# srtweezer/RobustGRAPE

Measured on AMD Instinct MI355X. Metric: GRAPE gradient-evals/sec (fidelity+∇), Rydberg CZ d=9 N_t=512, 1→8 GPU, higher is better.
Workload: dtype f64

## Files before the change

### robustgrape_amd/csrc/grape_call.hip

```cpp
#include <hip/hip_runtime.h>

#include <algorithm>
#include <cstring>
#include <string>
#include <vector>

#include "grape_plan.hpp"

using namespace grape_eng;

namespace grape_eng {

static grape_dense::DenseBatch dense_batch(grape_plan *p, int nb, const double *d_x, double *d_F, double *d_Fdx,
                                           double *d_Fd2, double *d_Fd2dx) {
    grape_dense::DenseBatch DB{};
    DB.nb = nb;
    DB.x = d_x;
    DB.E = p->dn_E;
    DB.Q = p->dn_Q;
    DB.Carry = p->dn_Carry;
    DB.M = p->dn_M;
    DB.Mc = p->dn_Mc;
    DB.Z = p->dn_Z;
    DB.Ub = p->dn_Ub;
// ... 69 lines not shown
        FA.Fd2dx = P.ne ? d_Fd2dx + (size_t)b * P.ne * nx : nullptr;
        HIPCHECK(grape_unitary::launch_fidelity(FA, st));
        mk(GRAPE_KERNEL_GRAD, 1);
    }
    return GRAPE_OK;
}

static KMark profiling_mark(grape_plan *p) {
    KMark mk;
    if (p->profiling) {
        mk.ctx = p;
        mk.fn = [](void *ctx, int k, int phase) {
            grape_plan *pl = static_cast<grape_plan *>(ctx);
            hipEvent_t e = pl->get_event();
            if (!e) return;
            (void)hipEventRecord(e, pl->cur_stream);
            if (phase == 0) {
                pl->pending.push_back({k, e, nullptr});
            } else {
                pl->pending.back().b = e;
            }
        };
    }
    return mk;
}

static int enqueue_wide(grape_plan *p, int nb, const double *d_x, double *d_F, double *d_Fdx) {
    hipStream_t st = p->stream;
    p->cur_stream = st;
    const KMark mk = profiling_mark(p);
    const int ma = p->merge_pa, mb = 1 - ma;
    DevProblem Pw[2] = {p->Ps[ma], p->Ps[mb]};
    DevBatch Bw[2]{};
    grape_proj::SectorHead H = p->SH;
    for (int i = 0; i < 2; ++i) {
        const int cl = i == 0 ? ma : mb;
        const grape_plan::SecBuf &sb = p->sb[cl];
        Pw[i].nchunks = 1;
        Pw[i].L = Pw[i].Nt;
        Bw[i].nb = nb * Pw[i].nsec;
        Bw[i].x = d_x;
        Bw[i].F = d_F;
        Bw[i].Fdx = d_Fdx;
        Bw[i].Ub = sb.Tc;
        Bw[i].Msec = sb.Carry;
        Bw[i].status = p->d_ctrl + 2;
        Bw[i].sink = p->d_sink;
        H.Ub[cl] = sb.Tc;
        H.Msec[cl] = sb.Carry;
    }
    H.alpha = 1;
    H.x = d_x;
    H.F = d_F;
    H.Fdx = d_Fdx;
    H.tgt_part = p->d_tgt_part;
    mk(GRAPE_KERNEL_WALK_FWD, 0);
    HIPCHECK(grape_walk::launch_merged_wide(0, Pw[0], Bw[0], Pw[1], Bw[1], st));
    mk(GRAPE_KERNEL_WALK_FWD, 1);
    mk(GRAPE_KERNEL_SCAN, 0);
    HIPCHECK(grape_proj::launch_sector_head(H, nb, st));
    mk(GRAPE_KERNEL_SCAN, 1);
    mk(GRAPE_KERNEL_WALK_GRAD, 0);
    HIPCHECK(grape_walk::launch_merged_wide(1, Pw[0], Bw[0], Pw[1], Bw[1], st));
    mk(GRAPE_KERNEL_WALK_GRAD, 1);
    return GRAPE_OK;
}

static int enqueue(grape_plan *p, int nb, const double *d_x, double *d_F, double *d_Fdx, double *d_Fd2,
                   double *d_Fd2dx) {
    hipStream_t st = p->stream;
    p->cur_stream = st;
    const KMark mk = profiling_mark(p);
    if (p->tiled) {
        grape_tiled::TiledBatch TB = p->TB;
        TB.nb = nb;
        TB.x = d_x;
        TB.F = d_F;
        TB.Fdx = d_Fdx;
        HIPCHECK(grape_tiled::launch_pipeline(p->TP, TB, st, mk));
        return GRAPE_OK;
    }
    if (p->general_h0) return enqueue_general(p, nb, d_x, d_F, d_Fdx, d_Fd2, d_Fd2dx, mk);
    if (p->dense) {
        const grape_dense::DenseBatch DB = dense_batch(p, nb, d_x, d_F, d_Fdx, d_Fd2, d_Fd2dx);
        HIPCHECK(grape_dense::launch_pipeline(p->DP, DB, st, mk));
        return GRAPE_OK;
    }
    if (p->e1) {
        mk(GRAPE_KERNEL_EVAL1, 0);
        HIPCHECK(grape_eval1::launch(eval1_args(p, d_x, d_F, d_Fdx), nb, st));
        mk(GRAPE_KERNEL_EVAL1, 1);
        return GRAPE_OK;
    }
// ... 509 lines not shown
```

### robustgrape_amd/csrc/grape_plan.hpp

```cpp
#pragma once
#include <hip/hip_runtime.h>

#include <string>
#include <vector>

#include "grape.h"
#include "grape_launch_api.hpp"
#include "grape_walk_api.hpp"
#include "grape_projector_api.hpp"
#include "grape_dense_api.hpp"
#include "grape_tiled_api.hpp"
#include "grape_unitary_api.hpp"
#include "grape_eval1_api.hpp"
#include "grape_plan_setup.hpp"
#include "grape_descriptor.hpp"

using grape::DevBatch;
using grape::DevProblem;
using grape::Term;
using grape_host::KMark;

#define HIPCHECK(expr)                                                                  \
    do {                                                                                \
        hipError_t e_ = (expr);                                                         \
// ... 63 lines not shown
    grape::FactorTab FT{};
    Term *d_fac_h0 = nullptr, *d_fac_err = nullptr;
    double *d_W = nullptr;
    cd *d_E = nullptr, *d_Q = nullptr, *d_Mc = nullptr, *d_Carry = nullptr, *d_Ub = nullptr, *d_Me = nullptr;
    grape::VSpec *d_vs = nullptr;
    int *d_ovf2 = nullptr;
    cd *d_ovf2_slots = nullptr;
    double *d_Fd2 = nullptr, *d_Fd2dx = nullptr, *d_part_err = nullptr;
    cd *d_Zl = nullptr;
    double *d_x = nullptr, *d_F = nullptr, *d_Fdx = nullptr, *d_part = nullptr, *d_tgt_part = nullptr;
    int *d_ovf = nullptr, *d_ctrl = nullptr;
    bool tables = false;
    cd *d_Htab = nullptr, *d_U0tab = nullptr;
    cd *d_sink = nullptr;
    cd *d_PA = nullptr, *d_PB = nullptr, *d_P0g = nullptr, *d_gpscr = nullptr;
    struct SecBuf {
        cd *E = nullptr, *Q = nullptr, *Mc = nullptr, *Carry = nullptr, *Ub = nullptr, *slots = nullptr,
           *ops = nullptr, *opsT = nullptr, *Msec = nullptr, *Tc = nullptr, *wscr = nullptr, *Ew = nullptr,
           *gEt = nullptr;
        int *ovf = nullptr, *ovf2 = nullptr, *sidx = nullptr, *gauge_n = nullptr;
        double *part = nullptr;
        cd *Zl = nullptr, *Me = nullptr, *TotS = nullptr, *MsecE = nullptr, *Wc = nullptr;
        double *part_err = nullptr;
    };
    int ncls = 0;
    DevProblem Ps[2]{};
    SecBuf sb[2];
    int *d_fixed = nullptr;
    grape_proj::SectorHead SH{};
    bool e1 = false;
    bool merged = false;
    int merge_pa = 0;
    int wide = 0;
    cd *d_e1_Et = nullptr, *d_e1_scr = nullptr;
    unsigned char *d_e1_tab = nullptr;
    int e1_pa = 0;
    long long *e1_trace = nullptr, *e1_trace_d = nullptr;
    double e1_phase[16] = {0};
    long e1_calls = 0;
    bool symmetry = false;
    cd *d_ops_sym = nullptr, *d_opsT_sym = nullptr, *d_PA_sym = nullptr, *d_PB_sym = nullptr;
    double *d_W_sym = nullptr;
    hipStream_t aux_stream = nullptr;
    hipEvent_t ev_fork = nullptr, ev_join = nullptr;
    bool capturing = false;
    bool dense = false;
    grape_dense::DenseProblem DP{};
    double *dn_opimg = nullptr, *dn_W = nullptr, *dn_E = nullptr, *dn_Q = nullptr, *dn_Carry = nullptr,
           *dn_M = nullptr, *dn_Mc = nullptr, *dn_Z = nullptr, *dn_Ub = nullptr, *dn_Zl = nullptr, *dn_Vc = nullptr,
           *dn_Sx = nullptr, *dn_Tot = nullptr, *dn_Me = nullptr, *dn_Mp = nullptr, *dn_B0 = nullptr,
           *dn_Fadd = nullptr, *dn_Fd2add = nullptr;
    bool tiled = false;
    grape_tiled::TiledProblem TP{};
    grape_tiled::TiledBatch TB{};
    int *tl_h_smax = nullptr;
    grape::VSpec *ud_vs = nullptr;
    cd *ud_E = nullptr, *ud_C = nullptr, *ud_V = nullptr, *ud_S = nullptr, *ud_out = nullptr;
    int *ud_ovf = nullptr;
    cd *ud_gscr = nullptr;
    bool general_h0 = false;
    bool pivot = false;
    cd *ud_Ci = nullptr, *d_G = nullptr;
    cd *d_fscr = nullptr;
    double *ud_Aimg = nullptr;
    std::vector<grape::VSpec> ud_vs_host;
    double *ud_Eimg = nullptr;
// ... 83 lines not shown
```

### robustgrape_amd/csrc/grape_plan_build.hip

```cpp
#include <hip/hip_runtime.h>

#include <algorithm>
#include <climits>
#include <cmath>
#include <cstdlib>
#include <cstring>
#include <string>
#include <vector>

#include "grape_plan.hpp"

namespace grape_eng {

static int merged_chunk_count(long MB, int Nt, int nc, int ncu) {
    if (const char *e = getenv("GRAPE_GAUGE_NCHUNKS")) {
        const int n = atoi(e);
        if (n > 0) return std::min(n, Nt);
    }
    const double simds = 4.0 * ncu;
    double best = 1e300;
    int pick = nc;
    for (int n = std::max(1, nc / 2); n <= std::min(2 * nc, Nt); ++n) {
        const int L = (Nt + n - 1) / n, nch = (Nt + L - 1) / L;
        const double waves = std::ceil((double)MB * nch / 64.0);
// ... 588 lines not shown
    *pb = 1;
    if (p->ncls == 2 && grape_walk::pair_ok(p->Ps[1], p->Ps[0])) std::swap(*pa, *pb);
}

static int setup_merge(PlanBuild &b) {
    grape_plan *p = b.p;
    if (p->ncls != 2) return GRAPE_OK;
    const DevProblem &P = p->P;
    int pa, pb;
    walk_pair_order(p, &pa, &pb);
    DevProblem &A = p->Ps[pa], &Bq = p->Ps[pb];
    if (!(grape_walk::pair_ok(A, Bq) && A.D == 3 && A.gauge && Bq.gauge && A.gauge_a == Bq.gauge_a &&
          A.scan_waves == kScanTiny && Bq.scan_waves == kScanTiny && A.nchunks <= Bq.nchunks && P.np == 1 && P.na <= 1))
        return GRAPE_OK;
    Bq.L = A.L;
    Bq.nchunks = A.nchunks;
    p->merged = !(P.opts & GRAPE_OPT_NO_MERGE) && grape_walk::merged_ok(A, Bq);
    p->merge_pa = pa;
    for (int cl = 0; p->merged && cl < 2; ++cl)
        if (int rc = fill_gauge_table(p, cl, false)) return rc;
    const std::vector<double> &W = b.sps().W;
    bool r1 = p->merged && p->SH.diag && !(P.opts & GRAPE_OPT_NO_RANK1);
    for (int cl = 0; cl < 2; ++cl) {
        const SectorClass &sc = b.ss.cls[cl];
        DevProblem &Pc = p->Ps[cl];
        Pc.rank1 = Pc.rank1_c[0] = Pc.rank1_c[1] = 0;
        r1 = r1 && sc.nsec <= 2;
        for (int w = 0; r1 && w < sc.nsec; ++w) {
            int n = 0;
            for (int r = 0; r < sc.S; ++r) {
                const int g = sc.sidx[(size_t)w * sc.S + r];
                if (g >= 0 && W[g] != 0.0) {
                    Pc.rank1_c[w] = r;
                    ++n;
                }
            }
            r1 = r1 && n == 1;
        }
        if (Pc.twin && grape_walk::merged_twin_sum()) r1 = r1 && Pc.rank1_c[0] == Pc.rank1_c[1];
    }
    A.rank1 = Bq.rank1 = r1 ? 1 : 0;
    const long wide = (long)p->max_batch * A.nchunks;
    if (r1 && !(P.opts & GRAPE_OPT_NO_WIDE) && grape_walk::wide_ok(A, Bq) && wide * 2 <= (long)INT_MAX) p->wide = (int)wide;
    return GRAPE_OK;
}

static int setup_eval1(grape_plan *p) {
    const grape_proj::SectorHead &H = p->SH;
    if (p->ncls != 2 || (long)p->max_batch > kEval1MaxBatch || (p->P.opts & GRAPE_OPT_NO_EVAL1)) return GRAPE_OK;
    int pa, pb;
    walk_pair_order(p, &pa, &pb);
    const DevProblem &A = p->Ps[pa], &Bq = p->Ps[pb];
    if (!grape_walk::pair_ok(A, Bq) || !grape_eval1::eligible(A, Bq, H)) return GRAPE_OK;
    if (p->mem.alloc(&p->d_e1_Et, (size_t)A.D * A.D + 8) != hipSuccess ||
        p->mem.alloc(&p->d_e1_scr, (size_t)2 * 2 * 16) != hipSuccess)
        return fail(GRAPE_ERR_ALLOC, "device allocation failed (eval1)");
    const hipError_t e = grape_eval1::prepare(A, Bq, p->d_e1_Et, p->d_e1_Et + (size_t)A.D * A.D, p->d_e1_scr, p->stream);
    if (e != hipSuccess || hipStreamSynchronize(p->stream) != hipSuccess)
        return fail(GRAPE_ERR_HIP, "eval1 preparation failed");
    p->e1 = true;
    p->e1_pa = pa;
    const size_t tb = grape_eval1::tab_bytes(A, Bq, H);
    if (p->mem.alloc(&p->d_e1_tab, std::max<size_t>(tb, 16)) != hipSuccess)
        return fail(GRAPE_ERR_ALLOC, "device allocation failed (eval1)");
    if (grape_eval1::tab_build(eval1_args(p, nullptr, nullptr, nullptr), p->d_e1_tab, p->stream) != hipSuccess ||
        hipStreamSynchronize(p->stream) != hipSuccess)
        return fail(GRAPE_ERR_HIP, "eval1 table build failed");
    const char *tr = std::getenv("GRAPE_EVAL1_TRACE");
    if (tr && tr[0] == '1' &&
        (hipHostMalloc(reinterpret_cast<void **>(&p->e1_trace), 32 * sizeof(long long), hipHostMallocDefault) != hipSuccess ||
         hipHostGetDevicePointer(reinterpret_cast<void **>(&p->e1_trace_d), p->e1_trace, 0) != hipSuccess))
        return fail(GRAPE_ERR_ALLOC, "eval1 trace buffer");
    return GRAPE_OK;
}

static int setup_sectors(PlanBuild &b) {
// ... 62 lines not shown
```

### robustgrape_amd/csrc/grape_projector.hip

```cpp
#include "grape_kernels.hpp"
#include "grape_projector_api.hpp"

namespace grape_proj {

namespace {

using grape::cd;
using grape::cadd, grape::csub, grape::cscale, grape::cmul, grape::cconj;
constexpr int BLOCK = 256;

template <bool H>
__device__ __forceinline__ cd el(const cd *X, int D, int i, int l) {
    return H ? cconj(X[(size_t)l * D + i]) : X[(size_t)i * D + l];
}

template <bool HA, bool HB>
__device__ void bmm(cd *C, const cd *A, const cd *B, int D) {
    for (int t = threadIdx.x; t < D * D; t += blockDim.x) {
        const int i = t / D, j = t % D;
        cd s{0.0, 0.0};
        for (int l = 0; l < D; ++l) s = cadd(s, cmul(el<HA>(A, D, i, l), el<HB>(B, D, l, j)));
        C[t] = s;
    }
    __syncthreads();
// ... 619 lines not shown
    if (ok && row == 0) H.F[b] = (fsum + tau.re * tau.re + tau.im * tau.im) / P.DD;
    double unused = 0.0;
    cd unused_c{0.0, 0.0};
    if (ok) diag_row_any(H, St, row, el, b, 1, u0, d, tau, unused, unused_c);
    for (int q = 0; q < P.na; ++q) {
        const grape::Pert pq = xadd_pert(P, q);
        __syncthreads();
        if (ok)
            for (int k = row; k < P.n_tgt; k += G) cq[k] = grape::term_coef(St.terms[k], 1, xb, xadd, pq);
        __syncthreads();
        if (ok)
            for (int i = row; i < P.D; i += G) d[i] = cscale(P.inv_eps, csub(target_entry(P, St, cq, i), u0[i]));
        __syncthreads();
        double sa = 0.0;
        cd trd{0.0, 0.0};
        if (ok) diag_row_any(H, St, row, el, b, 2, u0, d, tau, sa, trd);
        sa = group_add(sa, G);
        trd.re = group_add(trd.re, G);
        trd.im = group_add(trd.im, G);
        for (int r = 0; r < H.nfixed; ++r) {
            const int g = St.fixed[r];
            const cd kd = cconj(d[g]), k = cconj(u0[g]);
            sa += St.W[g] * (St.W[g] != 0.0 ? 1.0 : 0.0) * (kd.re * k.re + kd.im * k.im);
            trd = cadd(trd, cscale(St.W[g], kd));
        }
        const double val = (2.0 * sa + 2.0 * (tau.re * trd.re + tau.im * trd.im)) / P.DD;
        if (ok && row == 0) {
            if (P.xadd_dep && H.tgt_part) H.tgt_part[b * P.na + q] = val;
            else H.Fdx[b * P.nx + (size_t)P.np * P.Nt + q] = val;
        }
    }
}

template <int S>
__device__ void err_row(const SectorHead &H, int cl, int w, int r, size_t b, int e, int pass, const cd *u0, const cd *d,
                        cd te, cd *ue, double &t1, double &t2, cd &acc) {
    const grape::DevProblem &P = H.P;
    const int ns = H.nsec[cl], ne = P.ne;
    const double sc = 2.0 / P.DD;
    const size_t bw = b * ns + w;
    const cd *Ub = H.Ub[cl] + bw * S * S;
    int g[S];
#pragma unroll
    for (int k = 0; k < S; ++k) g[k] = H.sidx[cl][w * S + k];
    const int gr = g[r];
    auto cu0 = [&](int k) { return cconj(u0[g[k] >= 0 ? g[k] : 0]); };
    if (pass == 0) {
        const cd *Tb = H.TotS[cl] + (bw * ne + e) * S * S;
        cd Ur[S];
#pragma unroll
        for (int c = 0; c < S; ++c) {
            cd v{0.0, 0.0};
#pragma unroll
            for (int m = 0; m < S; ++m) v = cadd(v, cmul(Ub[r * S + m], Tb[m * S + c]));
            Ur[c] = (gr >= 0 && g[c] >= 0) ? v : cd{0.0, 0.0};
            ue[r * S + c] = Ur[c];
        }
        if (gr < 0) return;
        const double wr = P.W[gr];
#pragma unroll
        for (int c = 0; c < S; ++c) {
            if (g[c] < 0) continue;
            const cd ke = cmul(cu0(r), Ur[c]);
            t1 += wr * pdiag(P, g[c]) * (ke.re * ke.re + ke.im * ke.im);
            t2 += P.W[g[c]] * (Ur[c].re * Ur[c].re + Ur[c].im * Ur[c].im);
        }
// ... 94 lines not shown
        sa = group_add(sa, G);
        trd.re = group_add(trd.re, G);
        trd.im = group_add(trd.im, G);
        if (ok && row == 0)
            H.Fd2dx[(size_t)be * P.nx + (size_t)P.np * P.Nt + q] = 2.0 * (2.0 * sa + 2.0 * (te.re * trd.re + te.im * trd.im)) / P.DD;
    }
}

hipError_t launch_sector_err_head(const SectorHead &H, int nb, hipStream_t st) {
    if (H.P.ne == 0) return hipSuccess;
    if (H.diag) {
        const int G = diag_group(H), EB = kDiagBlock / G, n = nb * H.P.ne;
        const size_t lds = (size_t)EB * err_rows_group_cd(H) * sizeof(cd);
        hipLaunchKernelGGL(k_sec_err_head_rows, dim3((unsigned)((n + EB - 1) / EB)), dim3(kDiagBlock), lds, st, H, nb);
        return hipGetLastError();
    }
    const size_t lds = (size_t)kErrHeadSlots * H.P.D * H.P.D * sizeof(cd);
    hipLaunchKernelGGL(k_sec_err_head, dim3((unsigned)(nb * H.P.ne)), dim3(SEC_BLOCK), lds, st, H);
    return hipGetLastError();
}

hipError_t launch_sector_head(const SectorHead &H, int nb, hipStream_t st) {
    if (H.diag) {
        const DiagLayout L = diag_layout(H);
        hipLaunchKernelGGL(k_sec_head_diag, dim3((unsigned)((nb + L.EB - 1) / L.EB)), dim3(kDiagBlock), L.total, st, H,
                           nb);
        return hipGetLastError();
    }
    const size_t lds = (size_t)kHeadSlots * H.P.D * H.P.D * sizeof(cd);
    hipLaunchKernelGGL(k_sec_head, dim3((unsigned)nb), dim3(SEC_BLOCK), lds, st, H);
    return hipGetLastError();
}

hipError_t launch_fid_head(const Heads &H, int nb, hipStream_t st) {
    hipLaunchKernelGGL(k_proj_fid, dim3((unsigned)nb), dim3(BLOCK), 0, st, H);
    return hipGetLastError();
}

hipError_t launch_err_head(const Heads &H, int nb, hipStream_t st) {
    if (H.P.ne == 0) return hipSuccess;
    hipLaunchKernelGGL(k_proj_err, dim3((unsigned)(nb * H.P.ne)), dim3(BLOCK), 0, st, H);
    return hipGetLastError();
}

}
```

### robustgrape_amd/csrc/grape_projector_api.hpp

```cpp
#pragma once
#include <hip/hip_runtime.h>

#include "grape_types.hpp"

namespace grape_proj {

constexpr int kScratchSlots = 16;
constexpr size_t kImg = 2 * 64 * 64;

struct Heads {
    grape::DevProblem P;
    int dense;
    const double *x;
    const grape::cd *U0tab;
    const grape::cd *Ub;
    const grape::cd *Carry;
    grape::cd *Mc;
    grape::cd *Me;
    const double *Ub_img, *Tot_img;
    double *M_img, *Me_img;
    double *F, *Fdx, *tgt_part, *Fd2, *Fd2dx;
    grape::cd *scr;
};

hipError_t launch_fid_head(const Heads &H, int nb, hipStream_t st);
hipError_t launch_err_head(const Heads &H, int nb, hipStream_t st);

constexpr int kDiagMaxRows = 32;
struct SectorHead {
    grape::DevProblem P;
    int ncls;
    int S[2], nsec[2];
    const int *sidx[2];
    const grape::cd *Ub[2];
    grape::cd *Msec[2];
    const int *fixed;
    int nfixed;
    const double *x;
    double *F, *Fdx, *tgt_part;
    const grape::cd *TotS[2];
    grape::cd *MsecE[2];
    double *Fd2, *Fd2dx;
    int diag;
    int alpha;
};
hipError_t launch_sector_head(const SectorHead &H, int nb, hipStream_t st);
hipError_t launch_sector_err_head(const SectorHead &H, int nb, hipStream_t st);

inline Heads small_heads(const grape::DevProblem &P, const grape::DevBatch &B) {
    Heads H{};
    H.P = P;
    H.dense = 0;
    H.x = B.x;
    H.U0tab = B.U0tab;
    H.Ub = B.Ub;
    H.Carry = B.Carry;
    H.Mc = B.Mc;
    H.Me = B.Me;
    H.F = B.F;
    H.Fdx = B.Fdx;
    H.tgt_part = B.tgt_part;
    H.Fd2 = B.Fd2;
    H.Fd2dx = B.Fd2dx;
    H.scr = B.gp_scr;
    return H;
}

}
```

### robustgrape_amd/csrc/grape_walk_gauge.hpp

```cpp
#pragma once
#include "grape_cis.hpp"
#include "grape_walk_core.hpp"

namespace grape {

template <int D>
struct GaugeN {
    int n[D];
};
template <int D>
constexpr int kGaugePairs = D > 1 ? D * (D - 1) / 2 : 1;
__host__ __device__ constexpr int gauge_pair(int D, int j, int k) {
    return j * D - j * (j + 1) / 2 + (k - j - 1);
}
template <int D>
__device__ __forceinline__ GaugeN<D> gauge_charges(const DevProblem &P, int w) {
    const cptr<int> g = as_constant(P.gauge_n) + (size_t)w * D;
    GaugeN<D> r;
#pragma unroll
    for (int j = 0; j < D; ++j) r.n[j] = g[j];
    return r;
}
__device__ __forceinline__ cd gauge_pow(cd z, int n) {
    cd r = cmake(1.0, 0.0);
    if (n > 0) r = z;
#pragma unroll 1
    for (int m = 1; m < n; ++m) r = cmulf(r, z);
    return r;
}
struct CisConst {
    __device__ __forceinline__ double operator()(int i) const {
        double v = grape_cis::kCisCoef[i];
        asm("" : "+s"(v));
        return v;
    }
};
__device__ __forceinline__ cd gauge_cis(double t) {
    double s, c;
    if (fabs(t) <= grape_cis::kCisFast) grape_cis::cis_fast(t, s, c, CisConst());
    else sincos(t, &s, &c);
    return cmake(c, s);
}
static __device__ const grape_cis::CisTabEntry kCisTableDev[grape_cis::kCisTabN] = {GRAPE_CIS_TABLE_ENTRIES};
__device__ __forceinline__ void gauge_cis_stage(grape_cis::CisTabEntry *tab) {
    for (int i = threadIdx.x; i < grape_cis::kCisTabN; i += blockDim.x) tab[i] = kCisTableDev[i];
    __syncthreads();
}
__device__ __forceinline__ cd gauge_cis_tab(double t, const grape_cis::CisTabEntry *tab) {
    double s, c;
    if (fabs(t) <= grape_cis::kCisTabFast) grape_cis::cis_tab(t, tab, s, c, CisConst());
    else sincos(t, &s, &c);
    return cmake(c, s);
}
__device__ __forceinline__ double sin_small(double t) {
    const double t2 = t * t;
    return t * fma(t2, fma(t2, fma(t2, fma(t2, 1.0 / 362880.0, -1.0 / 5040.0), 1.0 / 120.0), -1.0 / 6.0), 1.0);
}
__device__ __forceinline__ cd cis_m1(double phi) {
    if (fabs(phi) <= 0.05) {
        const double sh = sin_small(0.5 * phi);
        return cmake(-2.0 * sh * sh, sin_small(phi));
    }
    const double sh = sin(0.5 * phi);
    return cmake(-2.0 * sh * sh, sin(phi));
}
template <int D>
__device__ __forceinline__ void gauge_fd_weights_dn(cd q, const GaugeN<D> &g, cd (&f)[kGaugePairs<D>]) {
#pragma unroll
    for (int r = 0; r < D; ++r) {
#pragma unroll
        for (int j = r + 1; j < D; ++j) {
            const int dn = g.n[r] - g.n[j], m = dn < 0 ? -dn : dn;
            cd z = q;
#pragma unroll 1
            for (int i = 1; i < m; ++i) z = cadd(cadd(z, q), cmulf(q, z));
            f[gauge_pair(D, r, j)] = m == 0 ? czero() : cmake(z.re, dn < 0 ? -z.im : z.im);
        }
    }
}
template <int D>
__device__ __forceinline__ cd gauge_fd_weight(const cd (&f)[kGaugePairs<D>], int r, int j) {
    return r < j ? f[gauge_pair(D, r, j)] : cconj(f[gauge_pair(D, j, r)]);
}
template <int D, int NE>
__device__ __forceinline__ void gauge_base(const DevProblem &P, cptr<cd> ops, cd *scr, cd (&Et)[NE][D][D]) {
    __shared__ cd gE[NE * D * D];
    if ((int)threadIdx.x < NE) {
        const int w = threadIdx.x;
        WalkX X0;
        X0.k0 = X0.k1 = X0.a0 = X0.a1 = 0.0;
        Pert none;
        none.var = -1;
        none.index = 0;
        none.delta = 0.0;
        SM<D> A[1];
        walk_build<D, 1>(P, ops + (size_t)w * P.sec_ops, X0, 1, none, A);
        double mu0 = 0.0;
// ... 87 lines not shown
```

### robustgrape_amd/csrc/grape_walk_merged.hpp

```cpp
#pragma once
#include "grape_walk_core.hpp"
#include "grape_walk_gauge.hpp"

namespace grape {

template <int D, bool SMEM>
__device__ __forceinline__ void gauge_prop_lds(const cd *Et, const cd (&e)[kGaugePairs<D>],
                                               MStore<D, false> &E) {
    if constexpr (SMEM) {
        cptr<cd> g = as_constant(Et);
        asm volatile("" : "+s"(g));
#pragma unroll
        for (int j = 0; j < D; ++j) {
#pragma unroll
            for (int k = 0; k < D; ++k) E.set(j, k, gauge_sandwich<D>(e, j, k, cload(g, j * D + k)));
        }
    } else {
#pragma unroll
        for (int j = 0; j < D; ++j) {
#pragma unroll
            for (int k = 0; k < D; ++k) E.set(j, k, gauge_sandwich<D>(e, j, k, Et[j * D + k]));
        }
    }
}
// ... 72 lines not shown
        }
#pragma unroll
        for (int j = 0; j < D; ++j) psi[w][j] = t[j];
    }
}
template <int D, int NE, int DP>
__device__ __forceinline__ void wide_reframe(const cd (&pw)[DP], cd (&chi)[NE][D]) {
    static_assert(D <= DP, "powers up to the sector's highest charge");
#pragma unroll
    for (int w = 0; w < NE; ++w) {
#pragma unroll
        for (int j = 1; j < D; ++j) chi[w][j] = cmulf(chi[w][j], pw[j]);
    }
}
template <int D, int NE>
__device__ __forceinline__ void wide_step_frame(const cd *Et, cd (&chi)[NE][D]) {
#pragma unroll
    for (int w = 0; w < NE; ++w) {
        cptr<cd> g = as_constant(Et + w * D * D);
        asm volatile("" : "+s"(g));
        cd t[D];
#pragma unroll
        for (int j = 0; j < D; ++j) {
            cd c = czero();
#pragma unroll
            for (int m = 0; m < D; ++m) cmac(c, chi[w][m], cload(g, j * D + m));
            t[j] = c;
        }
#pragma unroll
        for (int j = 0; j < D; ++j) chi[w][j] = t[j];
    }
}
template <int D>
__device__ __forceinline__ void wide_store_u(cd *u, int c, const cd (&psi)[D]) {
#pragma unroll
    for (int j = 0; j < D; ++j) {
#pragma unroll
        for (int i = 0; i < D; ++i) u[j * D + i] = i == c ? psi[j] : czero();
    }
}
constexpr int kFdxTile = 16;
__device__ __forceinline__ void wide_load_x(double (*tile)[kFdxTile + 1], const double *x, int nx, int nbe, int j0, int Nt) {
    constexpr int kStep = kWalkBlock / kFdxTile;
    const int j = threadIdx.x % kFdxTile, r0 = threadIdx.x / kFdxTile;
    const double *xc = x + min(j0 + j, Nt - 1);
    const long b0 = (long)blockIdx.x * kWalkBlock;
#pragma unroll 4
    for (int r = r0; r < kWalkBlock; r += kStep) tile[r][j] = xc[(size_t)min(b0 + r, (long)nbe - 1) * nx];
}
__device__ __forceinline__ bool wide_group_full(int nbe) {
    return GRAPE_WIDE_TILE_FAST && ((long)blockIdx.x + 1) * kWalkBlock <= (long)nbe;
}
__device__ __forceinline__ unsigned wide_tile_offset(int nx) {
    return (unsigned)((threadIdx.x / kFdxTile) * nx + threadIdx.x % kFdxTile) * (unsigned)sizeof(double);
}
__device__ __forceinline__ void wide_load_x_full(double (*tile)[kFdxTile + 1], const double *xb, int nx, unsigned off) {
    constexpr int kStep = kWalkBlock / kFdxTile, kTrips = kWalkBlock / kStep;
    const int j = threadIdx.x % kFdxTile, r0 = threadIdx.x / kFdxTile;
    double v[kTrips];
#pragma unroll
    for (int i = 0; i < kTrips; ++i)
        v[i] = *reinterpret_cast<const double *>(reinterpret_cast<const char *>(xb + (size_t)i * kStep * nx) + off);
#pragma unroll
    for (int i = 0; i < kTrips; ++i) tile[r0 + i * kStep][j] = v[i];
}
__device__ __forceinline__ void wide_flush_full(const double (*tile)[kFdxTile + 1], double *fb, int nx, unsigned off) {
    constexpr int kStep = kWalkBlock / kFdxTile, kTrips = kWalkBlock / kStep;
    const int j = threadIdx.x % kFdxTile, r0 = threadIdx.x / kFdxTile;
#pragma unroll
    for (int i = 0; i < kTrips; ++i)
        *reinterpret_cast<double *>(reinterpret_cast<char *>(fb + (size_t)i * kStep * nx) + off) = tile[r0 + i * kStep][j];
}
// ... 31 lines not shown
            wide_reframe<2, NEB>(pw, psiB);
            wide_step_frame<DA, 1>(PA.gauge_Et, psiA);
            wide_step_frame<2, NEB>(PB.gauge_Et, psiB);
        } else {
            wide_step_fwd<DA, 1, LAD>(PA.gauge_Et, gA, p1, psiA);
            wide_step_fwd<2, NEB, LAD>(PB.gauge_Et, gB, p1, psiB);
        }
    };
    const bool full = wide_group_full(L.nbe);
    const unsigned off = wide_tile_offset(PA.nx);
    const double *xb = BA.x + (size_t)blockIdx.x * kWalkBlock * PA.nx;
#pragma unroll 1
    for (int j0 = 0; j0 < PA.Nt; j0 += kFdxTile) {
        const int nj = min(kFdxTile, PA.Nt - j0);
        if (full && j0 + kFdxTile <= PA.Nt) wide_load_x_full(xtile, xb + j0, PA.nx, off);
        else wide_load_x(xtile, BA.x, PA.nx, L.nbe, j0, PA.Nt);
        __syncthreads();
        int t = 0;
#pragma unroll 1
        for (; t + 1 < nj; t += 2) {
            step(xtile[threadIdx.x][t]);
            step(xtile[threadIdx.x][t + 1]);
        }
        if (t < nj) step(xtile[threadIdx.x][t]);
        __syncthreads();
    }
    if constexpr (FRAME) {
        cd pw[DA];
        ladder_powers<DA>(pprev, pw);
        wide_reframe<DA, 1>(pw, psiA);
        wide_reframe<2, NEB>(pw, psiB);
    }
    if (L.ok) {
        wide_store_u<DA>(BA.Ub + (size_t)L.be * DA * DA, cA, psiA[0]);
#pragma unroll
        for (int w = 0; w < 2; ++w)
            wide_store_u<2>(BB.Ub + ((size_t)L.be * 2 + w) * 4, PB.rank1_c[w], psiB[TWB ? 0 : w]);
    }
}
template <int DA, bool TWB, bool LAD, bool WIDE = false>
__global__ __launch_bounds__(kWalkBlock, (WIDE ? GRAPE_WALK_WIDE_FWD_WAVES : GRAPE_WALK_FWD_M_WAVES)) void k_walk_fwd_m(DevProblem PA, DevBatch BA,
                                                                                  DevProblem PB, DevBatch BB) {
    if constexpr (WIDE) {
        wide_fwd_body<DA, TWB, LAD>(PA, BA, PB, BB);
        return;
    }
    constexpr int NEB = TWB ? 1 : 2;
    __shared__ grape_cis::CisTabEntry ctab[grape_cis::kCisTabN];
    gauge_cis_stage(ctab);
    const VBlock vb = hw_block();
    const WalkLane L = walk_lane<1>(PA, BA, vb);
    const double *xt = BA.x + (size_t)L.be * PA.nx;
    const cd *EtA = PA.gauge_Et, *EtB = PB.gauge_Et;
    GaugeN<DA> gA[1];
    GaugeN<2> gB[NEB];
    gA[0] = gauge_charges<DA>(PA, 0);
#pragma unroll
    for (int w = 0; w < NEB; ++w) gB[w] = gauge_charges<2>(PB, w);
    cd QA[1][DA][DA], QB[NEB][2][2];
#pragma unroll
    for (int j = 0; j < DA; ++j) {
#pragma unroll
        for (int i = 0; i < DA; ++i) QA[0][j][i] = cmake(i == j ? 1.0 : 0.0, 0.0);
    }
#pragma unroll
    for (int w = 0; w < NEB; ++w) {
#pragma unroll
        for (int j = 0; j < 2; ++j) {
#pragma unroll
            for (int i = 0; i < 2; ++i) QB[w][j][i] = cmake(i == j ? 1.0 : 0.0, 0.0);
// ... 319 lines not shown
                        c = fma(-z.im, g.im, c);
                    }
                }
            }
            const double sv = c * inv_eps;
            tot += sv;
            one = sv;
#pragma unroll
            for (int r = 0; r < D; ++r) {
                cd s = u[r][0];
#pragma unroll
                for (int j = 1; j < D; ++j) s = cadd(s, u[r][j]);
                psi[w][r] = s;
            }
        }
    }
    return NSEC > 1 ? tot : one;
}
template <int D>
__device__ __forceinline__ void merged_r1_init(const cd *ca, size_t nbe, const cd *Mw, const cd *Mw2, int c,
                                               cd (&psi)[D], cd (&phi)[D]) {
    cd m[D];
#pragma unroll
    for (int e = 0; e < D; ++e) m[e] = cconj(Mw2 ? cadd(Mw[c * D + e], Mw2[c * D + e]) : Mw[c * D + e]);
#pragma unroll
    for (int j = 0; j < D; ++j) {
        cd s = czero();
#pragma unroll
        for (int e = 0; e < D; ++e) cmac(s, ca[(size_t)(j * D + e) * nbe], m[e]);
        phi[j] = s;
        psi[j] = ca[(size_t)(j * D + c) * nbe];
    }
}
template <int D, int NE, int NSEC, bool LAD>
__device__ __forceinline__ double wide_step_grad(const cd *Et, const GaugeN<D> (&gn)[NE], cd p1, cd q, double inv_eps,
                                                 cd (&psi)[NSEC][D], cd (&phi)[NSEC][D]) {
    constexpr int NSH = NSEC / NE;
    MStore<D, false> E[NE];
#pragma unroll
    for (int w = 0; w < NE; ++w) {
        cd dph[kGaugePairs<D>];
        if constexpr (LAD) gauge_phases_ladder<D>(p1, dph);
        else gauge_phases<D>(p1, gn[w], dph);
        gauge_prop_lds<D, true>(Et + w * D * D, dph, E[w]);
    }
    cd rh[D];
    if constexpr (LAD) ladder_rho<D>(q, rh);
    double tot = 0.0, one = 0.0;
#pragma unroll
    for (int we = 0; we < NE; ++we) {
        cd fw[kGaugePairs<D>];
        if constexpr (!LAD) {
            gauge_fd_weights_dn<D>(q, gn[we], fw);
        }
#pragma unroll
        for (int t = 0; t < NSH; ++t) {
            const int w = we * NSH + t;
            cd pm[D], v[D][D];
#pragma unroll
            for (int j = 0; j < D; ++j) {
                cd s = czero();
#pragma unroll
                for (int r = 0; r < D; ++r) cmac(s, cconj(E[we].at(r, j)), psi[w][r]);
                pm[j] = s;
            }
#pragma unroll
            for (int r = 0; r < D; ++r) {
#pragma unroll
                for (int j = 0; j < D; ++j) v[r][j] = cmulf(cconj(phi[w][r]), E[we].at(r, j));
            }
            double c = 0.0;
            if constexpr (LAD) {
                double tre[D], tim[D];
#pragma unroll
                for (int m = 0; m < D; ++m) tre[m] = tim[m] = 0.0;
#pragma unroll
                for (int r = 0; r < D; ++r) {
#pragma unroll
                    for (int j = 0; j < D; ++j) {
                        if (r == j) continue;
                        const int m = r > j ? r - j : j - r;
                        tre[m] = fma(v[r][j].re, pm[j].re, tre[m]);
                        tre[m] = fma(-v[r][j].im, pm[j].im, tre[m]);
                        if (r > j) {
                            tim[m] = fma(v[r][j].re, pm[j].im, tim[m]);
                            tim[m] = fma(v[r][j].im, pm[j].re, tim[m]);
                        } else {
                            tim[m] = fma(-v[r][j].re, pm[j].im, tim[m]);
                            tim[m] = fma(-v[r][j].im, pm[j].re, tim[m]);
                        }
                    }
                }
#pragma unroll
                for (int m = 1; m < D; ++m) {
                    c = fma(rh[m].re, tre[m], c);
                    c = fma(-rh[m].im, tim[m], c);
                }
            } else {
#pragma unroll
                for (int r = 0; r < D; ++r) {
#pragma unroll
                    for (int j = 0; j < D; ++j) {
                        if (r == j) continue;
                        const cd z = cmulf(v[r][j], pm[j]), g = gauge_fd_weight<D>(fw, r, j);
                        c = fma(z.re, g.re, c);
                        c = fma(-z.im, g.im, c);
                    }
                }
            }
            const double sv = c * inv_eps;
            tot += sv;
            one = sv;
#pragma unroll
            for (int j = 0; j < D; ++j) {
                cd s = v[0][j];
#pragma unroll
                for (int r = 1; r < D; ++r) s = cadd(s, v[r][j]);
                phi[w][j] = cconj(s);
                psi[w][j] = pm[j];
            }
        }
    }
    return NSEC > 1 ? tot : one;
}
template <int D>
__device__ __forceinline__ void wide_grad_init(const cd *u, const cd *a, const cd *a2, int c, cd (&psi)[D], cd (&phi)[D]) {
    const cd al = cconj(a2 ? cadd(*a, *a2) : *a);
#pragma unroll
    for (int j = 0; j < D; ++j) {
        psi[j] = u[j * D + c];
        phi[j] = j == c ? al : czero();
    }
}
template <int DA, bool TWB, bool LAD>
__device__ __forceinline__ void wide_grad_body(const DevProblem &PA, const DevBatch &BA, const DevProblem &PB,
                                               const DevBatch &BB, double (*ftile)[kFdxTile + 1], int2 *frow,
                                               const grape_cis::CisTabEntry *ctab) {
    constexpr int NEB = TWB ? 1 : 2;
    constexpr int NXB = (TWB && GRAPE_WALK_TWIN_SUM) ? 1 : 2;
    const WideLane L = wide_lane(BA);
    frow[threadIdx.x] = make_int2(L.ok ? L.be : -1, 0);
    cd psiA[1][DA], phiA[1][DA], psiB[NXB][2], phiB[NXB][2];
    const size_t be = (size_t)L.be;
    wide_grad_init<DA>(BA.Ub + be * DA * DA, BA.Msec + be, nullptr, PA.rank1_c[0], psiA[0], phiA[0]);
#pragma unroll
    for (int w = 0; w < NXB; ++w) {
        const cd *ab = BB.Msec + be * 2 + w;
        wide_grad_init<2>(BB.Ub + (be * 2 + w) * 4, ab, NXB == 1 ? ab + 1 : nullptr, PB.rank1_c[w], psiB[w], phiB[w]);
    }
    GaugeN<DA> gA[1];
    GaugeN<2> gB[NEB];
    gA[0] = gauge_charges<DA>(PA, 0);
#pragma unroll
    for (int w = 0; w < NEB; ++w) gB[w] = gauge_charges<2>(PB, w);
    auto step = [&](double xk) {
        const double xe = xk + PA.eps;
        const cd p1 = gauge_cis_tab(PA.gauge_a * xk, ctab), q = cis_m1(PA.gauge_a * (xe - xk));
        const double sa = wide_step_grad<DA, 1, 1, LAD>(PA.gauge_Et, gA, p1, q, PA.inv_eps, psiA, phiA);
        const double sb = wide_step_grad<2, NEB, NXB, LAD>(PB.gauge_Et, gB, p1, q, PB.inv_eps, psiB, phiB);
        return sa + sb;
    };
    const int jlast = (PA.Nt - 1) / kFdxTile * kFdxTile;
    const bool full = wide_group_full(L.nbe);
    const unsigned off = wide_tile_offset(PA.nx);
    const size_t row0 = (size_t)blockIdx.x * kWalkBlock * PA.nx;
#pragma unroll 1
    for (int j0 = jlast; j0 >= 0; j0 -= kFdxTile) {
        const int nj = min(kFdxTile, PA.Nt - j0);
        const bool fast = full && j0 + kFdxTile <= PA.Nt;
        if (fast) wide_load_x_full(ftile, BA.x + row0 + j0, PA.nx, off);
        else wide_load_x(ftile, BA.x, PA.nx, L.nbe, j0, PA.Nt);
        __syncthreads();
#pragma unroll 1
        for (int t = nj - 1; t >= 0; --t) ftile[threadIdx.x][t] = step(ftile[threadIdx.x][t]);
        __syncthreads();
        if (fast) {
            wide_flush_full(ftile, BA.Fdx + row0 + j0, PA.nx, off);
        } else {
            const int j = threadIdx.x % kFdxTile;
#pragma unroll 1
            for (int row = threadIdx.x / kFdxTile; row < kWalkBlock; row += kWalkBlock / kFdxTile) {
                const int br = frow[row].x;
                if (j < nj && br >= 0) BA.Fdx[(size_t)br * PA.nx + j0 + j] = ftile[row][j];
            }
        }
        __syncthreads();
    }
}
template <int DA, bool TWB, bool LAD, bool R1, bool WIDE = false>
__global__ __launch_bounds__(kWalkBlock, (WIDE ? GRAPE_WALK_WIDE_GRAD_WAVES : R1 ? GRAPE_WALK_R1_WAVES : GRAPE_WALK_MERGED_WAVES)) void k_walk_grad_m(DevProblem PA, DevBatch BA,
                                                                                   DevProblem PB, DevBatch BB) {
    constexpr int NEB = TWB ? 1 : 2;
// ... 89 lines not shown
```

Baseline: 127.2 million.

## Add dedicated wide head kernel, compact psi storage, linearize FD weights

```diff
diff --git a/robustgrape_amd/csrc/grape_call.hip b/robustgrape_amd/csrc/grape_call.hip
--- a/robustgrape_amd/csrc/grape_call.hip
+++ b/robustgrape_amd/csrc/grape_call.hip
@@ -125,7 +125,6 @@
     const int ma = p->merge_pa, mb = 1 - ma;
     DevProblem Pw[2] = {p->Ps[ma], p->Ps[mb]};
     DevBatch Bw[2]{};
-    grape_proj::SectorHead H = p->SH;
     for (int i = 0; i < 2; ++i) {
         const int cl = i == 0 ? ma : mb;
         const grape_plan::SecBuf &sb = p->sb[cl];
@@ -139,19 +138,32 @@
         Bw[i].Msec = sb.Carry;
         Bw[i].status = p->d_ctrl + 2;
         Bw[i].sink = p->d_sink;
-        H.Ub[cl] = sb.Tc;
-        H.Msec[cl] = sb.Carry;
-    }
-    H.alpha = 1;
+    }
+    grape_proj::WideHead H{};
+    H.P = p->SH.P;
+    H.fixed = p->SH.fixed;
+    H.nfixed = p->SH.nfixed;
     H.x = d_x;
     H.F = d_F;
     H.Fdx = d_Fdx;
-    H.tgt_part = p->d_tgt_part;
+    int ns = 0;
+    for (int cl = 0; cl < 2; ++cl) {
+        const DevProblem &Pc = p->Ps[cl];
+        for (int w = 0; w < Pc.nsec; ++w, ++ns) {
+            if (ns == 3) return fail(GRAPE_ERR_HIP, "wide pass: more than three sectors");
+            const int ch = (cl == mb && Pc.twin) ? 0 : w;
+            H.lev[ns] = p->wide_lev[cl][w];
+            H.ucc[ns] = p->sb[cl].Tc + ((size_t)ch * Pc.D + Pc.rank1_c[w]) * nb;
+            H.alpha[ns] = p->sb[cl].Carry + w;
+            H.astride[ns] = Pc.nsec;
+        }
+    }
+    if (ns != 3) return fail(GRAPE_ERR_HIP, "wide pass: fewer than three sectors");
     mk(GRAPE_KERNEL_WALK_FWD, 0);
     HIPCHECK(grape_walk::launch_merged_wide(0, Pw[0], Bw[0], Pw[1], Bw[1], st));
     mk(GRAPE_KERNEL_WALK_FWD, 1);
     mk(GRAPE_KERNEL_SCAN, 0);
-    HIPCHECK(grape_proj::launch_sector_head(H, nb, st));
+    HIPCHECK(grape_proj::launch_wide_head(H, nb, st));
     mk(GRAPE_KERNEL_SCAN, 1);
     mk(GRAPE_KERNEL_WALK_GRAD, 0);
     HIPCHECK(grape_walk::launch_merged_wide(1, Pw[0], Bw[0], Pw[1], Bw[1], st));
diff --git a/robustgrape_amd/csrc/grape_fd_weight.hpp b/robustgrape_amd/csrc/grape_fd_weight.hpp
--- /dev/null
+++ b/robustgrape_amd/csrc/grape_fd_weight.hpp
@@ -0,0 +1,59 @@
+#pragma once
+
+#include <hip/hip_runtime.h>
+
+namespace grape_fd {
+
+struct Z {
+    double re, im;
+};
+
+__host__ __device__ __forceinline__ double sin_small(double t) {
+    const double t2 = t * t;
+    return t * fma(t2, fma(t2, fma(t2, fma(t2, 1.0 / 362880.0, -1.0 / 5040.0), 1.0 / 120.0), -1.0 / 6.0), 1.0);
+}
+__host__ __device__ __forceinline__ Z cis_m1(double phi) {
+    if (fabs(phi) <= 0.05) {
+        const double sh = sin_small(0.5 * phi);
+        return Z{-2.0 * sh * sh, sin_small(phi)};
+    }
+    const double sh = sin(0.5 * phi);
+    return Z{-2.0 * sh * sh, sin(phi)};
+}
+__host__ __device__ __forceinline__ Z rho_next(Z q, Z z) {
+    return Z{(z.re + q.re) + fma(q.re, z.re, -(q.im * z.im)), (z.im + q.im) + fma(q.re, z.im, q.im * z.re)};
+}
+__host__ __device__ __forceinline__ Z rho_pow(Z q, int m) {
+    Z z = q;
+    for (int i = 1; i < m; ++i) z = rho_next(q, z);
+    return z;
+}
+
+struct Base {
+    Z rho0, g;
+};
+__host__ __device__ __forceinline__ Base fd_base_signed(Z r, int dn) {
+    return Base{r, Z{-(double)dn * r.im, (double)dn * (1.0 + r.re)}};
+}
+__host__ __device__ __forceinline__ Base fd_base_from(Z rho_abs, int dn) {
+    if (dn == 0) return Base{Z{0.0, 0.0}, Z{0.0, 0.0}};
+    return fd_base_signed(Z{rho_abs.re, dn < 0 ? -rho_abs.im : rho_abs.im}, dn);
+}
+__host__ __device__ __forceinline__ Base fd_base(double phi0, int dn) {
+    return fd_base_from(rho_pow(cis_m1(phi0), dn < 0 ? -dn : dn), dn);
+}
+__host__ __device__ __forceinline__ double fd_threshold(double phi0, int m_max) {
+    const double p = fabs(phi0);
+    if (!(m_max >= 1) || !(p > 0.0) || !((double)m_max * p <= 0.5)) return -1.0;
+    return fmin(0.5 * p, sqrt(0x1p-55 * p) / (double)m_max);
+}
+__host__ __device__ __forceinline__ double fd_threshold_h(double a, double eps, int m_max) {
+    const double t = fd_threshold(a * eps, m_max);
+    return t < 0.0 ? -1.0 : t / fabs(a);
+}
+__host__ __device__ __forceinline__ Base fd_base_h(Base b, double a) { return Base{b.rho0, Z{a * b.g.re, a * b.g.im}}; }
+__host__ __device__ __forceinline__ Z fd_step(const Base &b, double d) {
+    return Z{fma(d, b.g.re, b.rho0.re), fma(d, b.g.im, b.rho0.im)};
+}
+
+}
diff --git a/robustgrape_amd/csrc/grape_plan.hpp b/robustgrape_amd/csrc/grape_plan.hpp
--- a/robustgrape_amd/csrc/grape_plan.hpp
+++ b/robustgrape_amd/csrc/grape_plan.hpp
@@ -119,6 +119,7 @@
     bool merged = false;
     int merge_pa = 0;
     int wide = 0;
+    int wide_lev[2][2] = {{0, 0}, {0, 0}};
     cd *d_e1_Et = nullptr, *d_e1_scr = nullptr;
     unsigned char *d_e1_tab = nullptr;
     int e1_pa = 0;
diff --git a/robustgrape_amd/csrc/grape_plan_build.hip b/robustgrape_amd/csrc/grape_plan_build.hip
--- a/robustgrape_amd/csrc/grape_plan_build.hip
+++ b/robustgrape_amd/csrc/grape_plan_build.hip
@@ -644,6 +644,7 @@
                 const int g = sc.sidx[(size_t)w * sc.S + r];
                 if (g >= 0 && W[g] != 0.0) {
                     Pc.rank1_c[w] = r;
+                    p->wide_lev[cl][w] = g;
                     ++n;
                 }
             }
@@ -653,7 +654,9 @@
     }
     A.rank1 = Bq.rank1 = r1 ? 1 : 0;
     const long wide = (long)p->max_batch * A.nchunks;
-    if (r1 && !(P.opts & GRAPE_OPT_NO_WIDE) && grape_walk::wide_ok(A, Bq) && wide * 2 <= (long)INT_MAX) p->wide = (int)wide;
+    if (r1 && !(P.opts & GRAPE_OPT_NO_WIDE) && grape_walk::wide_ok(A, Bq) && wide * 2 <= (long)INT_MAX &&
+        p->SH.nfixed <= grape_proj::kWideHeadMaxFixed)
+        p->wide = (int)wide;
     return GRAPE_OK;
 }
 
diff --git a/robustgrape_amd/csrc/grape_projector.hip b/robustgrape_amd/csrc/grape_projector.hip
--- a/robustgrape_amd/csrc/grape_projector.hip
+++ b/robustgrape_amd/csrc/grape_projector.hip
@@ -675,6 +675,98 @@
     }
 }
 
+template <class T>
+using cptr = const __attribute__((address_space(4))) T *;
+constexpr int kWideHeadBlock = 64, kWideHeadLevels = 3 + kWideHeadMaxFixed;
+__global__ __launch_bounds__(kWideHeadBlock) void k_wide_head(WideHead H, int nb) {
+    const grape::DevProblem &P = H.P;
+    const long gl = (long)blockIdx.x * kWideHeadBlock + threadIdx.x;
+    if (gl >= (long)nb) return;
+    const size_t b = (size_t)gl;
+    const double *xb = H.x + b * P.nx, *xadd = xb + (size_t)P.np * P.Nt;
+    const cptr<double> Wc = (cptr<double>)P.W;
+    const cptr<int> fx = (cptr<int>)H.fixed;
+    const cptr<cd> ops = (cptr<cd>)P.ops;
+    const cptr<grape::Term> terms = (cptr<grape::Term>)P.tgt;
+    constexpr int NL = kWideHeadLevels;
+    int g[NL];
+    double W[NL];
+#pragma unroll
+    for (int l = 0; l < NL; ++l) {
+        g[l] = l < 3 ? H.lev[l] : (l - 3 < H.nfixed ? fx[l - 3 < H.nfixed ? l - 3 : 0] : -1);
+        W[l] = g[l] >= 0 ? Wc[g[l]] : 0.0;
+    }
+    cd u0[NL], u1[NL];
+#pragma unroll
+    for (int l = 0; l < NL; ++l) u0[l] = u1[l] = cd{0.0, 0.0};
+    const grape::Pert none = no_pert(), pq = xadd_pert(P, 0);
+    for (int q = 0; q < P.n_tgt; ++q) {
+        grape::Term tm;
+        tm.op = terms[q].op;
+        tm.var = terms[q].var;
+        tm.index = terms[q].index;
+        tm.func = terms[q].func;
+        tm.a = terms[q].a;
+        tm.b = terms[q].b;
+        tm.sre = terms[q].sre;
+        tm.sim = terms[q].sim;
+        const cd c0 = grape::term_coef(tm, 1, xb, xadd, none);
+        const cd c1 = P.na ? grape::term_coef(tm, 1, xb, xadd, pq) : c0;
+#pragma unroll
+        for (int l = 0; l < NL; ++l) {
+            if (g[l] < 0) continue;
+            const size_t at = ((size_t)tm.op * P.D + g[l]) * P.D + g[l];
+            const cd o{ops[at].re, ops[at].im};
+            u0[l] = cadd(u0[l], cmul(c0, o));
+            u1[l] = cadd(u1[l], cmul(c1, o));
+        }
+    }
+    auto pd = [](double w) { return w != 0.0 ? 1.0 : 0.0; };
+    cd U[3], K[3];
+    double fsum = 0.0;
+    cd tau{0.0, 0.0};
+#pragma unroll
+    for (int s = 0; s < 3; ++s) {
+        U[s] = H.ucc[s][b];
+        K[s] = cmul(cconj(u0[s]), U[s]);
+        fsum += W[s] * pd(W[s]) * (K[s].re * K[s].re + K[s].im * K[s].im);
+        tau = cadd(tau, cscale(W[s], K[s]));
+    }
+#pragma unroll
+    for (int l = 3; l < NL; ++l) {
+        if (g[l] < 0) continue;
+        const cd k = cconj(u0[l]);
+        fsum += W[l] * pd(W[l]) * (k.re * k.re + k.im * k.im);
+        tau = cadd(tau, cscale(W[l], k));
+    }
+    H.F[b] = (fsum + tau.re * tau.re + tau.im * tau.im) / P.DD;
+    const double sc = 2.0 / P.DD;
+#pragma unroll
+    for (int s = 0; s < 3; ++s) {
+        const cd f = cadd(cscale(pd(W[s]), cconj(K[s])), cd{tau.re, -tau.im});
+        H.alpha[s][b * (size_t)H.astride[s]] = cscale(sc, cscale(W[s], cmul(cconj(u0[s]), f)));
+    }
+    if (P.na) {
+        double sa = 0.0;
+        cd trd{0.0, 0.0};
+#pragma unroll
+        for (int s = 0; s < 3; ++s) {
+            const cd dr = cconj(cscale(P.inv_eps, csub(u1[s], u0[s])));
+            const cd kd = cmul(dr, U[s]);
+            sa += W[s] * pd(W[s]) * (kd.re * K[s].re + kd.im * K[s].im);
+            trd = cadd(trd, cscale(W[s], kd));
+        }
+#pragma unroll
+        for (int l = 3; l < NL; ++l) {
+            if (g[l] < 0) continue;
+            const cd kd = cconj(cscale(P.inv_eps, csub(u1[l], u0[l]))), k = cconj(u0[l]);
+            sa += W[l] * pd(W[l]) * (kd.re * k.re + kd.im * k.im);
+            trd = cadd(trd, cscale(W[l], kd));
+        }
+        H.Fdx[b * P.nx + (size_t)P.np * P.Nt] = (2.0 * sa + 2.0 * (tau.re * trd.re + tau.im * trd.im)) / P.DD;
+    }
+}
+
 template <int S>
 __device__ void err_row(const SectorHead &H, int cl, int w, int r, size_t b, int e, int pass, const cd *u0, const cd *d,
                         cd te, cd *ue, double &t1, double &t2, cd &acc) {
@@ -835,6 +927,15 @@
     return hipGetLastError();
 }
 
+hipError_t launch_wide_head(const WideHead &H, int nb, hipStream_t st) {
+    const grape::DevProblem &P = H.P;
+    if (nb < 1 || P.na > 1 || P.xadd_dep || P.ne != 0 || H.nfixed < 0 || H.nfixed > kWideHeadMaxFixed) return hipErrorInvalidValue;
+    for (int s = 0; s < 3; ++s)
+        if (H.lev[s] < 0 || H.lev[s] >= P.D || !H.ucc[s] || !H.alpha[s]) return hipErrorInvalidValue;
+    hipLaunchKernelGGL(k_wide_head, dim3((unsigned)((nb + kWideHeadBlock - 1) / kWideHeadBlock)), dim3(kWideHeadBlock), 0, st, H, nb);
+    return hipGetLastError();
+}
+
 hipError_t launch_fid_head(const Heads &H, int nb, hipStream_t st) {
     hipLaunchKernelGGL(k_proj_fid, dim3((unsigned)nb), dim3(BLOCK), 0, st, H);
     return hipGetLastError();
diff --git a/robustgrape_amd/csrc/grape_projector_api.hpp b/robustgrape_amd/csrc/grape_projector_api.hpp
--- a/robustgrape_amd/csrc/grape_projector_api.hpp
+++ b/robustgrape_amd/csrc/grape_projector_api.hpp
@@ -47,6 +47,20 @@
 hipError_t launch_sector_head(const SectorHead &H, int nb, hipStream_t st);
 hipError_t launch_sector_err_head(const SectorHead &H, int nb, hipStream_t st);
 
+constexpr int kWideHeadMaxFixed = 5;
+struct WideHead {
+    grape::DevProblem P;
+    int lev[3];
+    const grape::cd *ucc[3];
+    grape::cd *alpha[3];
+    int astride[3];
+    const int *fixed;
+    int nfixed;
+    const double *x;
+    double *F, *Fdx;
+};
+hipError_t launch_wide_head(const WideHead &H, int nb, hipStream_t st);
+
 inline Heads small_heads(const grape::DevProblem &P, const grape::DevBatch &B) {
     Heads H{};
     H.P = P;
diff --git a/robustgrape_amd/csrc/grape_walk_gauge.hpp b/robustgrape_amd/csrc/grape_walk_gauge.hpp
--- a/robustgrape_amd/csrc/grape_walk_gauge.hpp
+++ b/robustgrape_amd/csrc/grape_walk_gauge.hpp
@@ -1,5 +1,6 @@
 #pragma once
 #include "grape_cis.hpp"
+#include "grape_fd_weight.hpp"
 #include "grape_walk_core.hpp"
 
 namespace grape {
@@ -52,17 +53,9 @@
     else sincos(t, &s, &c);
     return cmake(c, s);
 }
-__device__ __forceinline__ double sin_small(double t) {
-    const double t2 = t * t;
-    return t * fma(t2, fma(t2, fma(t2, fma(t2, 1.0 / 362880.0, -1.0 / 5040.0), 1.0 / 120.0), -1.0 / 6.0), 1.0);
-}
 __device__ __forceinline__ cd cis_m1(double phi) {
-    if (fabs(phi) <= 0.05) {
-        const double sh = sin_small(0.5 * phi);
-        return cmake(-2.0 * sh * sh, sin_small(phi));
-    }
-    const double sh = sin(0.5 * phi);
-    return cmake(-2.0 * sh * sh, sin(phi));
+    const grape_fd::Z q = grape_fd::cis_m1(phi);
+    return cmake(q.re, q.im);
 }
 template <int D>
 __device__ __forceinline__ void gauge_fd_weights_dn(cd q, const GaugeN<D> &g, cd (&f)[kGaugePairs<D>]) {
diff --git a/robustgrape_amd/csrc/grape_walk_merged.hpp b/robustgrape_amd/csrc/grape_walk_merged.hpp
--- a/robustgrape_amd/csrc/grape_walk_merged.hpp
+++ b/robustgrape_amd/csrc/grape_walk_merged.hpp
@@ -128,12 +128,9 @@
     }
 }
 template <int D>
-__device__ __forceinline__ void wide_store_u(cd *u, int c, const cd (&psi)[D]) {
-#pragma unroll
-    for (int j = 0; j < D; ++j) {
-#pragma unroll
-        for (int i = 0; i < D; ++i) u[j * D + i] = i == c ? psi[j] : czero();
-    }
+__device__ __forceinline__ void wide_store_psi(cd *u, size_t nbe, const cd (&psi)[D]) {
+#pragma unroll
+    for (int j = 0; j < D; ++j) u[j * nbe] = psi[j];
 }
 constexpr int kFdxTile = 16;
 __device__ __forceinline__ void wide_load_x(double (*tile)[kFdxTile + 1], const double *x, int nx, int nbe, int j0, int Nt) {
@@ -231,10 +228,10 @@
         wide_reframe<2, NEB>(pw, psiB);
     }
     if (L.ok) {
-        wide_store_u<DA>(BA.Ub + (size_t)L.be * DA * DA, cA, psiA[0]);
-#pragma unroll
-        for (int w = 0; w < 2; ++w)
-            wide_store_u<2>(BB.Ub + ((size_t)L.be * 2 + w) * 4, PB.rank1_c[w], psiB[TWB ? 0 : w]);
+        wide_store_psi<DA>(BA.Ub + L.be, (size_t)L.nbe, psiA[0]);
+#pragma unroll
+        for (int w = 0; w < NEB; ++w)
+            wide_store_psi<2>(BB.Ub + (size_t)w * 2 * L.nbe + L.be, (size_t)L.nbe, psiB[w]);
     }
 }
 template <int DA, bool TWB, bool LAD, bool WIDE = false>
@@ -620,9 +617,11 @@
         psi[j] = ca[(size_t)(j * D + c) * nbe];
     }
 }
-template <int D, int NE, int NSEC, bool LAD>
-__device__ __forceinline__ double wide_step_grad(const cd *Et, const GaugeN<D> (&gn)[NE], cd p1, cd q, double inv_eps,
+template <int D, int NE, int NSEC, bool LAD, int DR>
+__device__ __forceinline__ double wide_step_grad(const cd *Et, const GaugeN<D> (&gn)[NE], cd p1, const cd (&rh)[DR],
+                                                 const cd (&fw)[NE][kGaugePairs<D>], double inv_eps,
                                                  cd (&psi)[NSEC][D], cd (&phi)[NSEC][D]) {
+    static_assert(D <= DR, "weights up to the sector's highest charge difference");
     constexpr int NSH = NSEC / NE;
     MStore<D, false> E[NE];
 #pragma unroll
@@ -632,15 +631,9 @@
         else gauge_phases<D>(p1, gn[w], dph);
         gauge_prop_lds<D, true>(Et + w * D * D, dph, E[w]);
     }
-    cd rh[D];
-    if constexpr (LAD) ladder_rho<D>(q, rh);
     double tot = 0.0, one = 0.0;
 #pragma unroll
     for (int we = 0; we < NE; ++we) {
-        cd fw[kGaugePairs<D>];
-        if constexpr (!LAD) {
-            gauge_fd_weights_dn<D>(q, gn[we], fw);
-        }
 #pragma unroll
         for (int t = 0; t < NSH; ++t) {
             const int w = we * NSH + t;
@@ -690,7 +683,7 @@
 #pragma unroll
                     for (int j = 0; j < D; ++j) {
                         if (r == j) continue;
-                        const cd z = cmulf(v[r][j], pm[j]), g = gauge_fd_weight<D>(fw, r, j);
+                        const cd z = cmulf(v[r][j], pm[j]), g = gauge_fd_weight<D>(fw[we], r, j);
                         c = fma(z.re, g.re, c);
                         c = fma(-z.im, g.im, c);
                     }
@@ -711,12 +704,88 @@
     }
     return NSEC > 1 ? tot : one;
 }
+__device__ __forceinline__ double wide_uniform(double v) {
+    const int lo = __builtin_amdgcn_readfirstlane(__double2loint(v)), hi = __builtin_amdgcn_readfirstlane(__double2hiint(v));
+    return __hiloint2double(hi, lo);
+}
+template <int DA, int NEB, bool LAD>
+struct WideFd {
+    static constexpr int NW = LAD ? DA - 1 : kGaugePairs<DA> + NEB;
+    double eps, thr;
+    grape_fd::Base b[NW];
+};
+template <int DA, int NEB, bool LAD>
+__device__ __forceinline__ void wide_fd_base(double a, double eps, const GaugeN<DA> (&gA)[1], const GaugeN<2> (&gB)[NEB],
+                                             WideFd<DA, NEB, LAD> &fd) {
+    static_assert(DA >= 2, "class B's pair reads rho(1)");
+    const cd q0 = cis_m1(a * eps);
+    int mmax = 0;
+    auto take = [&](int i, cd f, int dn) {
+        const grape_fd::Base b = grape_fd::fd_base_h(grape_fd::fd_base_signed(grape_fd::Z{f.re, f.im}, dn), a);
+        fd.b[i].rho0 = grape_fd::Z{wide_uniform(b.rho0.re), wide_uniform(b.rho0.im)};
+        fd.b[i].g = (LAD && NEB == 1) ? b.g : grape_fd::Z{wide_uniform(b.g.re), wide_uniform(b.g.im)};
+        mmax = max(mmax, dn < 0 ? -dn : dn);
+    };
+    if constexpr (LAD) {
+        cd rh0[DA];
+        ladder_rho<DA>(q0, rh0);
+#pragma unroll
+        for (int m = 1; m < DA; ++m) take(m - 1, rh0[m], m);
+    } else {
+        cd f0[kGaugePairs<DA>], f1[1];
+        gauge_fd_weights_dn<DA>(q0, gA[0], f0);
+#pragma unroll
+        for (int r = 0; r < DA; ++r) {
+#pragma unroll
+            for (int j = r + 1; j < DA; ++j) take(gauge_pair(DA, r, j), f0[gauge_pair(DA, r, j)], gA[0].n[r] - gA[0].n[j]);
+        }
+#pragma unroll
+        for (int w = 0; w < NEB; ++w) {
+            gauge_fd_weights_dn<2>(q0, gB[w], f1);
+            take(kGaugePairs<DA> + w, f1[0], gB[w].n[0] - gB[w].n[1]);
+        }
+    }
+    fd.eps = eps;
+    fd.thr = wide_uniform(grape_fd::fd_threshold_h(a, eps, mmax));
+}
+template <int DA, int NEB, bool LAD>
+__device__ __forceinline__ void wide_fd_weights(const WideFd<DA, NEB, LAD> &fd, double a, double h, const GaugeN<DA> (&gA)[1],
+                                                const GaugeN<2> (&gB)[NEB], cd (&rh)[DA], cd (&fwA)[1][kGaugePairs<DA>],
+                                                cd (&fwB)[NEB][1]) {
+    const double dh = h - fd.eps;
+    auto at = [&](int i) {
+        const grape_fd::Z z = grape_fd::fd_step(fd.b[i], dh);
+        return cmake(z.re, z.im);
+    };
+    if (fabs(dh) <= fd.thr) {
+        if constexpr (LAD) {
+            rh[0] = czero();
+#pragma unroll
+            for (int m = 1; m < DA; ++m) rh[m] = at(m - 1);
+        } else {
+#pragma unroll
+            for (int i = 0; i < kGaugePairs<DA>; ++i) fwA[0][i] = at(i);
+#pragma unroll
+            for (int w = 0; w < NEB; ++w) fwB[w][0] = at(kGaugePairs<DA> + w);
+        }
+    } else {
+        const cd q = cis_m1(a * h);
+        if constexpr (LAD) {
+            ladder_rho<DA>(q, rh);
+        } else {
+            gauge_fd_weights_dn<DA>(q, gA[0], fwA[0]);
+#pragma unroll
+            for (int w = 0; w < NEB; ++w) gauge_fd_weights_dn<2>(q, gB[w], fwB[w]);
+        }
+    }
+}
 template <int D>
-__device__ __forceinline__ void wide_grad_init(const cd *u, const cd *a, const cd *a2, int c, cd (&psi)[D], cd (&phi)[D]) {
+__device__ __forceinline__ void wide_grad_init(const cd *u, size_t nbe, const cd *a, const cd *a2, int c, cd (&psi)[D],
+                                               cd (&phi)[D]) {
     const cd al = cconj(a2 ? cadd(*a, *a2) : *a);
 #pragma unroll
     for (int j = 0; j < D; ++j) {
-        psi[j] = u[j * D + c];
+        psi[j] = u[j * nbe];
         phi[j] = j == c ? al : czero();
     }
 }
@@ -730,22 +799,28 @@
     frow[threadIdx.x] = make_int2(L.ok ? L.be : -1, 0);
     cd psiA[1][DA], phiA[1][DA], psiB[NXB][2], phiB[NXB][2];
     const size_t be = (size_t)L.be;
-    wide_grad_init<DA>(BA.Ub + be * DA * DA, BA.Msec + be, nullptr, PA.rank1_c[0], psiA[0], phiA[0]);
+    const size_t nbe = (size_t)L.nbe;
+    wide_grad_init<DA>(BA.Ub + be, nbe, BA.Msec + be, nullptr, PA.rank1_c[0], psiA[0], phiA[0]);
 #pragma unroll
     for (int w = 0; w < NXB; ++w) {
         const cd *ab = BB.Msec + be * 2 + w;
-        wide_grad_init<2>(BB.Ub + (be * 2 + w) * 4, ab, NXB == 1 ? ab + 1 : nullptr, PB.rank1_c[w], psiB[w], phiB[w]);
+        wide_grad_init<2>(BB.Ub + (size_t)(TWB ? 0 : w) * 2 * nbe + be, nbe, ab, NXB == 1 ? ab + 1 : nullptr, PB.rank1_c[w],
+                          psiB[w], phiB[w]);
     }
     GaugeN<DA> gA[1];
     GaugeN<2> gB[NEB];
     gA[0] = gauge_charges<DA>(PA, 0);
 #pragma unroll
     for (int w = 0; w < NEB; ++w) gB[w] = gauge_charges<2>(PB, w);
+    WideFd<DA, NEB, LAD> fd;
+    wide_fd_base<DA, NEB, LAD>(PA.gauge_a, PA.eps, gA, gB, fd);
     auto step = [&](double xk) {
         const double xe = xk + PA.eps;
-        const cd p1 = gauge_cis_tab(PA.gauge_a * xk, ctab), q = cis_m1(PA.gauge_a * (xe - xk));
-        const double sa = wide_step_grad<DA, 1, 1, LAD>(PA.gauge_Et, gA, p1, q, PA.inv_eps, psiA, phiA);
-        const double sb = wide_step_grad<2, NEB, NXB, LAD>(PB.gauge_Et, gB, p1, q, PB.inv_eps, psiB, phiB);
+        const cd p1 = gauge_cis_tab(PA.gauge_a * xk, ctab);
+        cd rh[DA], fwA[1][kGaugePairs<DA>], fwB[NEB][1];
+        wide_fd_weights<DA, NEB, LAD>(fd, PA.gauge_a, xe - xk, gA, gB, rh, fwA, fwB);
+        const double sa = wide_step_grad<DA, 1, 1, LAD>(PA.gauge_Et, gA, p1, rh, fwA, PA.inv_eps, psiA, phiA);
+        const double sb = wide_step_grad<2, NEB, NXB, LAD>(PB.gauge_Et, gB, p1, rh, fwB, PB.inv_eps, psiB, phiB);
         return sa + sb;
     };
     const int jlast = (PA.Nt - 1) / kFdxTile * kFdxTile;
```

Result: faster. 137.7 million, median of 6 (+8.2%).
